# alexklibisz/deep-calcium

Hardware: NVIDIA B200
Metric: UNet2DS 512x512 images/sec (8x TTA) (higher is better)
Workload: dtype f16

## Files before the change

### deep-calcium_b200/csrc/core.cu

```cuda
#include "common.cuh"

namespace dcb {

unsigned long long g_launches = 0;

char* last_error_buf() {
  static thread_local char buf[512] = {0};
  return buf;
}

int fail(int code, const char* fmt, ...) {
  va_list ap;
  va_start(ap, fmt);
  vsnprintf(last_error_buf(), 512, fmt, ap);
  va_end(ap);
  return code;
}

int sm_count() {
  static int cached = 0;
  if (cached == 0) {
    int dev = 0, n = 0;
    if (cudaGetDevice(&dev) == cudaSuccess &&
        cudaDeviceGetAttribute(&n, cudaDevAttrMultiProcessorCount, dev) == cudaSuccess && n > 0)
      cached = n;
    else
      cached = 148;
  }
  return cached;
}

static const int kPolicyDefaults[DCB_POLICY_COUNT] = {
     1,  1,  1,  1,  64,  1,
     4,  0,  1,  2,  1,  1,  0,  0};
static int g_policy[DCB_POLICY_COUNT] = {1, 1, 1, 1, 64, 1, 4, 0, 1, 2, 1, 1, 0, 0};

int policy(int key) { return (key >= 0 && key < DCB_POLICY_COUNT) ? g_policy[key] : 0; }

char* last_kernel_buf() {
  static thread_local char buf[96] = {0};
  return buf;
}
void note_kernel(const char* name) {
  char* b = last_kernel_buf();
  strncpy(b, name, 95);
  b[95] = 0;
}

}

// ... 20 lines not shown
```

### deep-calcium_b200/csrc/tapgemm_tc.cu

```cuda
#include <cstdlib>
#include <mutex>
#include <map>
#include <vector>
#include <tuple>

#include "tc_common.cuh"
#include "stats_epilogue.cuh"
#include "tapgeom.h"

namespace dcb {
extern unsigned long long g_launches;
using namespace tc;

constexpr int TC_BM = 128;
constexpr int TC_MAX_STAGES = 8;
constexpr int TC_THREADS = 64 + 8 * 32;
constexpr int ST_QUARTETS = 2;
constexpr int ST_THREADS = 64 + ST_QUARTETS * 4 * 32;
constexpr int WG_THREADS = 192;

struct TcFusion {
  const float* head_kernel; const float* head_bias; float* logit; float* prob; int need_y; void* pool_out;
};

// ... 119 lines not shown
#pragma unroll
    for (int k = 0; k < 16; ++k) st[k * 32 + lane] = pooled[k];
    __syncwarp();
#pragma unroll
    for (int q = 0; q < 2; ++q) {
      const int idx = lane + 32 * q, pp = idx >> 2, chunk = idx & 3;
      const long long o = pool_index(m0 + 2 * pp);
      if (o >= 0)
        *reinterpret_cast<uint4*>(reinterpret_cast<uint16_t*>(pool_base) + o + chunk * 8) =
            *reinterpret_cast<const uint4*>(st + pp * 32 + chunk * 8);
    }
    __syncwarp();
  }
}

template <bool POOL, bool STATS>
__global__ void __launch_bounds__(TC_THREADS, 1)
tapgemm_tc_fwd_kernel(const __grid_constant__ CUtensorMap mapA0, const __grid_constant__ CUtensorMap mapA1,
                      const __grid_constant__ CUtensorMap mapB, const __grid_constant__ CUtensorMap mapO, const TcFwdParams p) {
  extern __shared__ __align__(1024) uint8_t smem_raw[];
  __shared__ uint64_t bar_full[TC_MAX_STAGES], bar_empty[TC_MAX_STAGES], bar_tfull[2], bar_tempty[2];
  __shared__ uint32_t tmem_base_smem;
  __shared__ __align__(16) float s_scale[512], s_shift[512];

  const int warp = threadIdx.x >> 5, lane = threadIdx.x & 31;
  if (threadIdx.x == 0) pdl_trigger();
  uint8_t* smem = smem_raw + ((1024u - (smem_u32(smem_raw) & 1023u)) & 1023u);
  const int PX = p.swap ? 256 : TC_BM;
  const uint32_t a_bytes = PX * p.BK * 2, b_bytes = (p.swap ? 128 : p.BN) * p.BK * 2;
  const uint32_t stage_bytes = a_bytes + b_bytes;
  const int kb0 = p.C0 / p.BK, kb1 = p.C1 / p.BK;
  const int kb_per_tap = kb0 + kb1;
  const int num_kb = p.ntaps * kb_per_tap;
  const int Ktap = p.C0 + p.C1;
  const int num_ntiles = p.swap ? (p.Ntot + 127) / 128 : p.Ntot / p.BN;
  const int num_mtiles = p.tiles_w * p.tiles_h * p.tiles_n;
  const int num_tiles = num_mtiles * num_ntiles;
  const int acc_cols = p.swap ? 256 : p.BN;
  uint32_t tmem_cols = 32;
  while (tmem_cols < 2u * acc_cols) tmem_cols <<= 1;
  __shared__ __align__(16) uint8_t s_stage[4][4096];
  float2 st_s[STATS ? 8 : 1], st_q[STATS ? 8 : 1];
#pragma unroll
  for (int i = 0; i < (STATS ? 8 : 1); ++i) { st_s[i] = make_float2(0.f, 0.f); st_q[i] = make_float2(0.f, 0.f); }

  for (int i = threadIdx.x; i < p.Cz; i += blockDim.x) {
    s_scale[i] = p.scale ? p.scale[i] : 1.f;
    s_shift[i] = p.shift ? p.shift[i] : 0.f;
  }
  if (warp == 0 && lane == 0) {
    tma_prefetch_desc(&mapA0);
    if (p.C1 > 0) tma_prefetch_desc(&mapA1);
    tma_prefetch_desc(&mapB);
    for (int s = 0; s < p.stages; ++s) { mbar_init(&bar_full[s], 1); mbar_init(&bar_empty[s], 1); }
    for (int s = 0; s < 2; ++s) { mbar_init(&bar_tfull[s], 1); mbar_init(&bar_tempty[s], 4); }
    mbar_fence_init();
  }
  if (warp == 1) {
    tmem_alloc(&tmem_base_smem, tmem_cols);
    tmem_relinquish();
  }
  tc_fence_before();
  __syncthreads();
  tc_fence_after();
  const uint32_t tmem_base = tmem_base_smem;

  if (warp == 0) {
    if (elect_one()) {
      int stage = 0; uint32_t phase = 0;
      pdl_wait();
      for (int tile = blockIdx.x; tile < num_tiles; tile += gridDim.x) {
        const int nt = tile % num_ntiles, mt = tile / num_ntiles;
        const int tw = mt % p.tiles_w, th = (mt / p.tiles_w) % p.tiles_h, tn = mt / (p.tiles_w * p.tiles_h);
        const int w0 = tw * p.bw, h0 = th * p.bh, n0 = tn * p.bn;
        for (int tap = 0; tap < p.ntaps; ++tap) {
          for (int kk = 0; kk < kb_per_tap; ++kk) {
            const bool second = kk >= kb0;
            const int c0 = (second ? kk - kb0 : kk) * p.BK;
            const CUtensorMap* mA = second ? &mapA1 : &mapA0;
            mbar_wait(&bar_empty[stage], phase ^ 1);
            uint8_t* sa = smem + (size_t)stage * stage_bytes;
            uint8_t* sb = sa + a_bytes;
            const int wrows = p.swap ? (p.Ntot - nt * 128 < 128 ? p.Ntot - nt * 128 : 128) : p.BN;
            mbar_arrive_expect_tx(&bar_full[stage], a_bytes + (uint32_t)wrows * p.BK * 2);
            if (p.mode == 0) tma_load_4d(mA, &bar_full[stage], sa, c0, w0 + p.dx[tap], h0 + p.dy[tap], n0);
            else if (p.mode == 1) tma_load_3d(mA, &bar_full[stage], sa, c0, w0, h0);
            else tma_load_5d(mA, &bar_full[stage], sa, c0, p.dx[tap], w0, p.dy[tap], h0);
            tma_load_2d(&mapB, &bar_full[stage], sb, tap * Ktap + (second ? p.C0 : 0) + c0, nt * (p.swap ? 128 : p.BN));
            if (++stage == p.stages) { stage = 0; phase ^= 1; }
          }
        }
      }
    }
  } else if (warp == 1) {
    if (elect_one()) {
      const uint32_t idesc = p.swap ? make_idesc_16(128, 256, 0, 0, p.f16) : make_idesc_16(TC_BM, p.BN, 0, 0, p.f16);
      const uint32_t swz = (p.BK == 64) ? SWZ_128B : SWZ_64B;
      const uint32_t sbo = 8u * p.BK * 2u;
      const int ksteps = p.BK / 16;
      const uint64_t dbase = make_smem_desc(0, 16, sbo, swz);
      const uint32_t smem16 = smem_u32(smem) >> 4, stage16 = stage_bytes >> 4, a16 = a_bytes >> 4;
      int stage = 0; uint32_t phase = 0;
      int acc = 0; uint32_t acc_phase = 0;
      const uint32_t a_full = smem_u32_pinned(bar_full), a_empty = smem_u32_pinned(bar_empty);
      asm volatile(".reg .pred p_full;");
      bool pre = false;
      for (int tile = blockIdx.x; tile < num_tiles; tile += gridDim.x) {
        mbar_wait(&bar_tempty[acc], acc_phase ^ 1);
        tc_fence_after();
        const uint32_t d_tmem = tmem_base + (uint32_t)(acc * acc_cols);
        for (int kb = 0; kb < num_kb; ++kb) {
          {
            uint32_t ok = 0;
            if (pre) asm volatile("selp.u32 %0, 1, 0, p_full;" : "=r"(ok));
            if (!ok) mbar_wait_a(a_full + 8u * stage, phase);
            int ns = stage + 1; uint32_t np = phase;
            if (ns == p.stages) { ns = 0; np ^= 1u; }
            asm volatile("mbarrier.test_wait.parity.shared::cta.b64 p_full, [%0], %1;" ::"r"(a_full + 8u * ns), "r"(np) : "memory");
            pre = true;
          }
          tc_fence_after();
          const uint32_t sa16 = smem16 + (uint32_t)stage * stage16, sb16 = sa16 + a16;
          const uint64_t da = dbase + (p.swap ? sb16 : sa16);
          const uint64_t db = dbase + (p.swap ? sa16 : sb16);
#pragma unroll
          for (int k = 0; k < 4; ++k) {
            if (k < ksteps) umma_bf16(d_tmem, da + (uint64_t)(2 * k), db + (uint64_t)(2 * k), idesc, (kb | k) != 0 ? 1u : 0u);
          }
          umma_commit_a(a_empty + 8u * stage);
          if (++stage == p.stages) { stage = 0; phase ^= 1; }
        }
        umma_commit(&bar_tfull[acc]);
        if (++acc == 2) { acc = 0; acc_phase ^= 1; }
      }
    }
  } else {
    const int quarter = warp & 3;
    const int m = quarter * 32 + lane;
    const int eset = (warp - 2) >> 2, nsets = p.swap ? 1 : 2;
    uint32_t it = 0;
    for (int tile = blockIdx.x; tile < num_tiles && eset < nsets; tile += gridDim.x, ++it) {
      if (nsets == 2 && (int)(it & 1u) != eset) continue;
      const int acc = (int)(it & 1u);
      const uint32_t acc_phase = (it >> 1) & 1u;
      const int nt = tile % num_ntiles, mt = tile / num_ntiles;
      const int tw = mt % p.tiles_w, th = (mt / p.tiles_w) % p.tiles_h, tn = mt / (p.tiles_w * p.tiles_h);
      if (p.swap) {
        const int grow = nt * 128 + quarter * 32;
        const bool warp_valid = grow < p.Ntot;
        const int z = grow / p.Cz, cw = grow % p.Cz;
        const int ody = p.Cz < p.Ntot ? (z >> 1) : p.ody, odx = p.Cz < p.Ntot ? (z & 1) : p.odx;
        const float sc = warp_valid ? s_scale[cw + lane] : 0.f, sh = warp_valid ? s_shift[cw + lane] : 0.f;
        auto pix_index = [&](int mm) -> long long {
          int n2, gh2, gw2;
          if (p.mode == 0) {
            gw2 = tw * p.bw + mm % p.bw;
            gh2 = th * p.bh + (mm / p.bw) % p.bh;
            n2 = tn * p.bn + mm / (p.bw * p.bh);
            if (gw2 >= p.GW || gh2 >= p.GH || n2 >= p.N) return -1;
          } else {
// ... 8 lines not shown
        tc_fence_after();
        if constexpr (POOL) {
          auto pool_index = [&](int mm) -> long long {
            const int gw2 = tw * p.bw + mm % p.bw, gh2 = th * p.bh + (mm / p.bw) % p.bh, n2 = tn * p.bn + mm / (p.bw * p.bh);
            if (gw2 >= p.GW || gh2 >= p.GH || n2 >= p.N) return -1;
            return (long long)((((size_t)n2 * (p.GH >> 1) + (gh2 >> 1)) * (p.GW >> 1) + (gw2 >> 1)) * p.OC + cw);
          };
          epilogue_swapped_pool(tmem_base + ((uint32_t)(quarter * 32) << 16) + (uint32_t)(acc * acc_cols), 256, p.bw, warp_valid, sc,
                                sh, p.relu, p.out, p.pool_out, s_stage[quarter], lane, pix_index, pool_index, p.f16);
        } else {
          epilogue_swapped(tmem_base + ((uint32_t)(quarter * 32) << 16) + (uint32_t)(acc * acc_cols), 256, warp_valid, sc, sh,
                           p.relu, p.out_f32, p.out, s_stage[quarter], lane, pix_index, p.f16);
        }
        tc_fence_before();
        __syncwarp();
        if (lane == 0) mbar_arrive(&bar_tempty[acc]);
        continue;
      }
      int n, gh, gw;
      bool valid;
      if (p.mode == 0) {
        gw = tw * p.bw + m % p.bw;
        gh = th * p.bh + (m / p.bw) % p.bh;
        n = tn * p.bn + m / (p.bw * p.bh);
        valid = gw < p.GW && gh < p.GH && n < p.N;
      } else {
        gw = tw * p.bw + m % p.bw;
        const int r = th * p.bh + m / p.bw;
        n = r / p.GH; gh = r % p.GH;
        valid = gw < p.GW && r < p.N * p.GH;
      }
// ... 137 lines not shown
              for (int q = 0; q < 4; ++q) {
                const uint4 b4 = stg[(m + 1) * 4 + q], c4 = stg[(m + p.bw) * 4 + q], d4 = stg[(m + p.bw + 1) * 4 + q];
                mx[4 * q] = max16x2(max16x2(pk[4 * q], b4.x, p.f16), max16x2(c4.x, d4.x, p.f16), p.f16);
                mx[4 * q + 1] = max16x2(max16x2(pk[4 * q + 1], b4.y, p.f16), max16x2(c4.y, d4.y, p.f16), p.f16);
                mx[4 * q + 2] = max16x2(max16x2(pk[4 * q + 2], b4.z, p.f16), max16x2(c4.z, d4.z, p.f16), p.f16);
                mx[4 * q + 3] = max16x2(max16x2(pk[4 * q + 3], b4.w, p.f16), max16x2(c4.w, d4.w, p.f16), p.f16);
              }
              store_pk16(p.pool_out + (((size_t)n * (p.GH >> 1) + (gh >> 1)) * (p.GW >> 1) + (gw >> 1)) * p.OC + cbase + c, mx);
            }
            asm volatile("bar.sync %0, 128;" ::"r"(1 + eset) : "memory");
          }
        }
      }
      tc_fence_before();
      __syncwarp();
      if (lane == 0) mbar_arrive(&bar_tempty[acc]);
    }
    if (p.tma_store && quarter == 0 && lane == 0) bulk_wait0();
  }

  tc_fence_before();
  __syncthreads();
  if (warp == 1) {
    tc_fence_after();
    tmem_dealloc(tmem_base, tmem_cols);
  }
  if constexpr (STATS) {
    float* dump = reinterpret_cast<float*>(smem);
    const int nblk = p.BN / 32;
    if (warp >= 2 && lane < 16) {
#pragma unroll
      for (int bi = 0; bi < 8; ++bi)
        if (bi < nblk)
          *reinterpret_cast<float4*>(dump + ((size_t)((warp - 2) * nblk + bi) * 16 + lane) * 4) =
              make_float4(st_s[bi].x, st_s[bi].y, st_q[bi].x, st_q[bi].y);
    }
    __syncthreads();
    const int nt = blockIdx.x % num_ntiles;
    stats_cta_finish(dump, 8, nblk, [&](int bi) { return (nt * p.BN + bi * 32) % p.Cz; }, p.Cz, p.stat_sums);
  }
// ... 46 lines not shown
  umma_bf16(d2, dA, dW + 2u * wblk16, id1, 0u);
  for (int kc = 0; kc < nkc; ++kc) {
#pragma unroll
    for (int dx = 0; dx < 3; ++dx) {
#pragma unroll
      for (int k = 0; k < KSTEPS; ++k) {
        if (kc == 0 && dx == 0 && k == 0) continue;
        umma_bf16(d0, dA + (kc * slot16 + dx * pitch16 + 2 * k), dW + ((uint32_t)(kc * 3 + dx) * 3u * wblk16 + 2 * k), id3, 1u);
      }
    }
  }
}

constexpr int ST_MAX_RING = 12;

__device__ __forceinline__ uint32_t cluster_ctarank() {
  uint32_t r;
  asm volatile("mov.u32 %0, %%cluster_ctarank;" : "=r"(r));
  return r;
}
__device__ __forceinline__ void cluster_sync_all() {
  asm volatile("barrier.cluster.arrive.release.aligned;" ::: "memory");
  asm volatile("barrier.cluster.wait.acquire.aligned;" ::: "memory");
}
__device__ __forceinline__ void tma_load_4d_mc(const CUtensorMap* m, uint64_t* bar, void* dst, int c0, int c1, int c2, int c3,
                                               uint16_t cta_mask) {
  asm volatile(
      "cp.async.bulk.tensor.4d.shared::cluster.global.mbarrier::complete_tx::bytes.multicast::cluster [%0], [%1, {%3, %4, %5, %6}], [%2], %7;"
      ::"r"(smem_u32(dst)), "l"(reinterpret_cast<uint64_t>(m)), "r"(smem_u32(bar)), "r"(c0), "r"(c1), "r"(c2), "r"(c3), "h"(cta_mask)
      : "memory");
}
__device__ __forceinline__ void umma_commit_mc2(uint32_t bar_addr) {
  asm volatile("tcgen05.commit.cta_group::1.mbarrier::arrive::one.shared::cluster.multicast::cluster.b64 [%0], %1;"
               ::"r"(bar_addr), "h"((uint16_t)3) : "memory");
}

#ifdef DCB_STRIP_TIMING
__device__ unsigned long long g_strip_dbg[148 * 8];
__device__ unsigned long long g_strip_dbg2[148 * 16];
// ... 641 lines not shown
    if (warp >= 2 && lane < 16) {
#pragma unroll
      for (int bi = 0; bi < 2; ++bi)
        if (bi < nblk)
          *reinterpret_cast<float4*>(dump + ((size_t)((warp - 2) * nblk + bi) * 16 + lane) * 4) =
              make_float4(sst.s[bi].x, sst.s[bi].y, sst.q[bi].x, sst.q[bi].y);
    }
    __syncthreads();
    stats_cta_finish(dump, 8, nblk, [](int bi) { return bi * 32; }, p.Cout, p.stat_sums);
  }
}

__device__ __forceinline__ uint32_t st2_region(int t0, int run) {
  return run == 3 ? 7u : (run == 2 ? (t0 == 0 ? 3u : 5u) : (uint32_t)t0);
}
__device__ __forceinline__ uint32_t mapa_u32(uint32_t addr, uint32_t rank) {
  uint32_t r;
  asm volatile("mapa.shared::cluster.u32 %0, %1, %2;" : "=r"(r) : "r"(addr), "r"(rank));
  return r;
}
__device__ __forceinline__ void mbar_arrive_cluster(uint32_t bar_addr) {
  asm volatile("mbarrier.arrive.relaxed.cluster.shared::cluster.b64 _, [%0];" ::"r"(bar_addr) : "memory");
}
__device__ __forceinline__ void mbar_arrive_expect_tx_cluster(uint32_t bar_addr, uint32_t bytes) {
  asm volatile("mbarrier.arrive.expect_tx.relaxed.cluster.shared::cluster.b64 _, [%0], %1;" ::"r"(bar_addr), "r"(bytes) : "memory");
}
__device__ __forceinline__ void tma_load_2d_pair(const CUtensorMap* m, uint32_t bar_addr, void* dst, int c0, int c1) {
  asm volatile(
      "cp.async.bulk.tensor.2d.shared::cluster.global.mbarrier::complete_tx::bytes.cta_group::2 [%0], [%1, {%3, %4}], [%2];"
      ::"r"(smem_u32(dst)), "l"(reinterpret_cast<uint64_t>(m)), "r"(bar_addr), "r"(c0), "r"(c1) : "memory");
}
__device__ __forceinline__ void tma_load_4d_pair(const CUtensorMap* m, uint32_t bar_addr, void* dst, int c0, int c1, int c2, int c3) {
  asm volatile(
      "cp.async.bulk.tensor.4d.shared::cluster.global.mbarrier::complete_tx::bytes.cta_group::2 [%0], [%1, {%3, %4, %5, %6}], [%2];"
      ::"r"(smem_u32(dst)), "l"(reinterpret_cast<uint64_t>(m)), "r"(bar_addr), "r"(c0), "r"(c1), "r"(c2), "r"(c3) : "memory");
}
__device__ __forceinline__ void umma2_bf16(uint32_t tmem_d, uint64_t desc_a, uint64_t desc_b, uint32_t idesc, uint32_t accumulate) {
  asm volatile(
      "{\n\t.reg .pred p;\n\t"
      "setp.ne.b32 p, %4, 0;\n\t"
      "tcgen05.mma.cta_group::2.kind::f16 [%0], %1, %2, %3, p;\n\t}"
      ::"r"(tmem_d), "l"(desc_a), "l"(desc_b), "r"(idesc), "r"(accumulate) : "memory");
}
__device__ __forceinline__ void umma2_commit_both(uint32_t bar_addr) {
  asm volatile("tcgen05.commit.cta_group::2.mbarrier::arrive::one.shared::cluster.multicast::cluster.b64 [%0], %1;"
               ::"r"(bar_addr), "h"((uint16_t)3) : "memory");
}

template <int KSTEPS>
__device__ __forceinline__ void fold2_issue_fast(uint32_t d0, uint32_t d2, uint64_t dA, uint64_t dW, uint32_t id1, uint32_t id2,
                                                 uint32_t id3, int nkc, uint32_t slot16, uint32_t pitch16, uint32_t half16,
                                                 uint32_t group16) {
  umma2_bf16(d0, dA, dW + 3u * half16, id2, 1u);
  umma2_bf16(d2, dA, dW + 2u * half16, id1, 0u);
  const uint64_t dW3 = dW + 7u * half16;
  for (int kc = 0; kc < nkc; ++kc) {
#pragma unroll
    for (int dx = 0; dx < 3; ++dx) {
#pragma unroll
      for (int k = 0; k < KSTEPS; ++k) {
        if (kc == 0 && dx == 0 && k == 0) continue;
        umma2_bf16(d0, dA + (kc * slot16 + dx * pitch16 + 2 * k), dW3 + ((uint32_t)(kc * 3 + dx) * group16 + 2 * k), id3, 1u);
// ... 28 lines not shown

  for (int i = threadIdx.x; i < p.Cout; i += blockDim.x) {
    s_scale[i] = p.scale ? p.scale[p.n0 + i] : 1.f;
    s_shift[i] = p.shift ? p.shift[p.n0 + i] : 0.f;
    s_wd[i] = p.head_kernel ? p.head_kernel[2 * i + 1] - p.head_kernel[2 * i] : 0.f;
  }
  if (warp == 0 && lane == 0) {
    tma_prefetch_desc(&mapA0);
    if (p.C1 > 0) tma_prefetch_desc(&mapA1);
    tma_prefetch_desc(&mapBh);
    mbar_init(&bar_w, 2);
    for (int s = 0; s < ring_pairs; ++s) { mbar_init(&row_full[s], 2); mbar_init(&row_empty[s], 1); }
    for (int s = 0; s < (nacc >> 1); ++s) { mbar_init(&bar_tfull[s], 1); mbar_init(&bar_tempty[s], 8); }
    mbar_fence_init();
  }
  if (warp == 1) {
    asm volatile("tcgen05.alloc.cta_group::2.sync.aligned.shared::cta.b32 [%0], %1;" ::"r"(smem_u32(&tmem_base_smem)), "r"(512u) : "memory");
    asm volatile("tcgen05.relinquish_alloc_permit.cta_group::2.sync.aligned;" ::: "memory");
  }
  tc_fence_before();
  cluster_sync_all();
  tc_fence_after();
  const uint32_t tmem_base = tmem_base_smem;

  const int units_per_col = p.H >> 1;
  const int npairs = gridDim.x >> 1, pair = blockIdx.x >> 1;
  const long long units = (long long)(p.N * p.wsegs / 2) * units_per_col;
  const long long u_begin = units * pair / npairs, u_end = units * (pair + 1) / npairs;
  auto next_strip = [&](long long& u, int& n, int& h0, int& rows, int& w0) -> bool {
    if (u >= u_end) return false;
    const int pcol = (int)(u / units_per_col), hu = (int)(u - (long long)pcol * units_per_col);
    long long take = units_per_col - hu;
    if (take > u_end - u) take = u_end - u;
    const int col = 2 * pcol + (int)rank;
// ... 173 lines not shown
        const uint32_t ta = t_lane + (j & (uint32_t)(nacc - 1)) * (uint32_t)p.Cout, tb = ta + (uint32_t)p.Cout;
        const int bar_i = (int)(jp & pmask);
        mbar_wait(&bar_tfull[bar_i], (j >> nacc_sh) & 1u);
        tc_fence_after();
        strip_drain_pair<FUSED>(p, ta, tb, n, h0 + t, w0 + m, s_scale, s_shift, s_wd, head_b, lane, p.n0);
        tc_fence_before();
        __syncwarp();
        if (lane == 0) mbar_arrive_cluster(l_tempty + 8u * bar_i);
      }
    }
  }
  tc_fence_before();
  cluster_sync_all();
  if (warp == 1) {
    tc_fence_after();
    asm volatile("tcgen05.dealloc.cta_group::2.sync.aligned.b32 %0, %1;" ::"r"(tmem_base), "r"(512u) : "memory");
  }
}

struct TcFlatParams {
  int N, H, W, Wp;
  int C0, C1, nkc;
  int Cout, mtiles;
  int NT, ptiles;
  int R;
  int wrows;
  uint32_t pbuf_bytes;
  int relu, out_f32;
  int f16;
  void* out;
  const float* scale;
// ... 517 lines not shown
                e[1], e[0] / e[1], e[3], e[2] / e[3], e[4] / e[3], e[5] / e[3], e[6] / e[3], e[8], e[7] / e[8], e[9] / e[8], e[10] / e[8], e[11] / e[8]);
        fprintf(stderr, "[strip timing] per CTA: fast rows %.0f | cycles/row: row_full wait %.0f, tempty wait %.0f, issue %.0f, commit %.0f, "
                "total %.0f | loop cycles %.0f\n", a[5], a[0] / a[5], a[1] / a[5], a[2] / a[5], a[3] / a[5], a[4] / a[5], a[6]);
      }
#endif
      return DCB_OK;
    }
  }
  if (!(stats && stats->sums && policy(DCB_POLICY_FUSED_BN) == 2)) {
    const int e = run_tc_flat(g, s0, C0, s1, C1, B, Nout, out, scale, shift, relu, out_f32, st, stats);
    if (e != DCB_ERR_UNSUPPORTED) return e;
  }
  return run_tc_generic(g, s0, C0, s1, C1, B, Nout, out, Nout, scale, shift, relu, out_f32, st, nullptr, stats);
}

static int run_tc_generic(const TapGeom& g, const void* s0, int C0, const void* s1, int C1, const void* B, int Nout, void* out,
                          int out_pitch, const float* scale, const float* shift, int relu, int out_f32, cudaStream_t st,
                          void* pool_out, TcStats* stats) {
  TcFwdParams p;
  memset(&p, 0, sizeof(p));
  const int ntaps = g.ntaps;
  const bool convT_fwd = g.zsub > 1;
  const bool convT_dgrad = (g.sy == 2);
  p.mode = convT_fwd ? 1 : (convT_dgrad ? 2 : 0);
  p.N = g.N; p.GH = g.GH; p.GW = g.GW;
  p.ntaps = ntaps;
  for (int t = 0; t < ntaps; ++t) { p.dy[t] = g.dy[t]; p.dx[t] = g.dx[t]; }
  p.C0 = C0; p.C1 = C1;
  p.BK = (C0 % 64 == 0 && C1 % 64 == 0) ? 64 : 32;
  const int swz = p.BK * 2;
  p.Cz = Nout;
  p.Ntot = convT_fwd ? 4 * Nout : Nout;
  p.OH = g.OH; p.OW = g.OW; p.OC = out_pitch;
  p.osy = g.osy; p.osx = g.osx; p.ody = g.ody; p.odx = g.odx;
  p.relu = relu; p.out_f32 = out_f32; p.out = reinterpret_cast<__nv_bfloat16*>(out); p.scale = scale; p.shift = shift;
  p.f16 = g.f16;
  {
    const long long px = (long long)g.N * g.GH * g.GW;
    p.swap = (p.mode == 0 && !pool_out && !stats && swap_allowed(Nout) && px / 256 * cdiv(p.Ntot, 128) >= sm_count() / 2) ? 1 : 0;
  }
  const int TM = p.swap ? 256 : TC_BM;
  if (p.mode == 0) {
    p.bw = pick_pow2_box(g.GW, TM);
    if (pool_out && p.bw == TM && TM >= 4) p.bw = TM / 2;
    p.bh = pick_pow2_box(g.GH, TM / p.bw);
    p.bn = TM / (p.bw * p.bh);
    p.tiles_w = cdiv(g.GW, p.bw); p.tiles_h = cdiv(g.GH, p.bh); p.tiles_n = cdiv(g.N, p.bn);
  } else {
    p.bw = pick_pow2_box(g.GW, TM);
    p.bh = TM / p.bw; p.bn = 1;
    p.tiles_w = cdiv(g.GW, p.bw); p.tiles_h = cdiv((long long)g.N * g.GH, p.bh); p.tiles_n = 1;
  }
  const int num_mtiles = p.tiles_w * p.tiles_h * p.tiles_n;
  if (pool_out) {
    if (p.mode != 0 || out_f32 || (g.GH & 1) || (g.GW & 1) || (p.bw & 1) || (p.bh & 1) || (p.swap && p.bw % 32 != 0) || out_pitch != Nout)
      return fail(DCB_ERR_UNSUPPORTED, "fused max-pool not available for this layer shape");
    p.pool_out = reinterpret_cast<__nv_bfloat16*>(pool_out);
  }
  int BN = 32;
  {
    double best = 1e30;
    for (int cand : {256, 192, 128, 96, 64, 32}) {
      if (cand > p.Ntot || p.Ntot % cand != 0) continue;
      const long long tiles = (long long)num_mtiles * (p.Ntot / cand);
      const long long waves = (tiles + sm_count() - 1) / sm_count();
      const double cost = (double)waves * (cand <= 128 ? 89.0 : 89.0 + (cand - 128) * (39.0 / 128.0));
      if (cost < best - 1e-9) { best = cost; BN = cand; }
    }
  }
  if (p.swap) BN = p.Ntot < 128 ? p.Ntot : 128;
  p.BN = BN;
  const size_t stage_bytes = (size_t)TM * p.BK * 2 + (size_t)(p.swap ? 128 : BN) * p.BK * 2;
  const bool with_stats = stats && !pool_out && !out_f32 && p.mode != 2 && out_pitch == Nout && stats->sums;
  p.tma_store = (!p.swap && !out_f32 && !pool_out && !with_stats && p.mode != 2 &&
                 (policy(DCB_POLICY_TMA_STORE) >= 2 || (policy(DCB_POLICY_TMA_STORE) == 1 && p.mode == 1))) ? 1 : 0;
  const size_t staging = p.tma_store ? 2 * 16384 : 0;
  int stages = (int)((200 * 1024 - staging) / stage_bytes);
  if (stages > TC_MAX_STAGES) stages = TC_MAX_STAGES;
  if (stages < 2) return fail(DCB_ERR_UNSUPPORTED, "tile does not fit shared memory");
  p.stages = stages;
  const size_t dyn_smem = stages * stage_bytes + staging + 1024;

  CUtensorMap mA0, mA1, mB;
  auto make_src_map = [&](CUtensorMap* m, const void* ptr, int C) -> int {
    if (p.mode == 0) {
      uint64_t dims[4] = {(uint64_t)C, (uint64_t)g.IW, (uint64_t)g.IH, (uint64_t)g.N};
      uint64_t str[3] = {(uint64_t)C * 2, (uint64_t)g.IW * C * 2, (uint64_t)g.IH * g.IW * C * 2};
      uint32_t box[4] = {(uint32_t)p.BK, (uint32_t)p.bw, (uint32_t)p.bh, (uint32_t)p.bn};
      return make_map(m, ptr, 4, dims, str, box, swz);
// ... 4 lines not shown
      return make_map(m, ptr, 3, dims, str, box, swz);
    } else {
      uint64_t dims[5] = {(uint64_t)C, 2, (uint64_t)g.GW, 2, (uint64_t)g.N * g.GH};
      uint64_t str[4] = {(uint64_t)C * 2, (uint64_t)2 * C * 2, (uint64_t)g.IW * C * 2, (uint64_t)2 * g.IW * C * 2};
      uint32_t box[5] = {(uint32_t)p.BK, 1, (uint32_t)p.bw, 1, (uint32_t)p.bh};
      return make_map(m, ptr, 5, dims, str, box, swz);
    }
  };
  if (int e = make_src_map(&mA0, s0, C0)) return e;
  if (C1 > 0) { if (int e = make_src_map(&mA1, s1, C1)) return e; }
  else mA1 = mA0;
  {
    const int Ktot = ntaps * (C0 + C1);
    uint64_t dims[2] = {(uint64_t)Ktot, (uint64_t)p.Ntot};
    uint64_t str[1] = {(uint64_t)Ktot * 2};
    uint32_t box[2] = {(uint32_t)p.BK, (uint32_t)BN};
    if (int e = make_map(&mB, B, 2, dims, str, box, swz)) return e;
  }

  CUtensorMap mO = mB;
  if (p.tma_store) {
    if (p.mode == 0) {
      uint64_t dims[4] = {(uint64_t)Nout, (uint64_t)g.OW, (uint64_t)g.OH, (uint64_t)g.N};
      uint64_t str[3] = {(uint64_t)out_pitch * 2, (uint64_t)g.OW * out_pitch * 2, (uint64_t)g.OH * g.OW * out_pitch * 2};
      uint32_t box[4] = {32u, (uint32_t)p.bw, (uint32_t)p.bh, (uint32_t)p.bn};
      if (int e = make_map(&mO, out, 4, dims, str, box, 64)) return e;
    } else {
      uint64_t dims[5] = {(uint64_t)Nout, 2, (uint64_t)g.GW, 2, (uint64_t)g.N * g.GH};
      uint64_t str[4] = {(uint64_t)out_pitch * 2, (uint64_t)2 * out_pitch * 2, (uint64_t)g.OW * out_pitch * 2,
                         (uint64_t)2 * g.OW * out_pitch * 2};
      uint32_t box[5] = {32u, 1, (uint32_t)p.bw, 1, (uint32_t)p.bh};
      if (int e = make_map(&mO, out, 5, dims, str, box, 64)) return e;
    }
  }
  static bool attr_set = false;
  if (!attr_set) {
    cudaError_t e = cudaFuncSetAttribute(tapgemm_tc_fwd_kernel<false, false>, cudaFuncAttributeMaxDynamicSharedMemorySize, 206 * 1024);
    if (e == cudaSuccess) e = cudaFuncSetAttribute(tapgemm_tc_fwd_kernel<true, false>, cudaFuncAttributeMaxDynamicSharedMemorySize, 206 * 1024);
    if (e == cudaSuccess) e = cudaFuncSetAttribute(tapgemm_tc_fwd_kernel<false, true>, cudaFuncAttributeMaxDynamicSharedMemorySize, 206 * 1024);
    if (e != cudaSuccess) return fail(DCB_ERR_CUDA, "cudaFuncSetAttribute(max dynamic smem) failed: %s", cudaGetErrorString(e));
    attr_set = true;
  }
  const int num_ntiles = p.swap ? cdiv(p.Ntot, 128) : p.Ntot / BN;
  const int num_tiles = num_mtiles * num_ntiles;
  int grid = num_tiles < sm_count() ? num_tiles : sm_count();
  const bool pdl = policy(DCB_POLICY_PDL) != 0;
  if (with_stats) {
    grid -= grid % num_ntiles;
    if (grid >= num_ntiles) {
      p.stat_sums = stats->sums;
      const cudaError_t le = launch_k(tapgemm_tc_fwd_kernel<false, true>, grid, TC_THREADS, dyn_smem, st, pdl, mA0, mA1, mB, mO, p);
      if (le != cudaSuccess) return fail(DCB_ERR_CUDA, "launch of tapgemm_tc_fwd_kernel (stats) failed: %s", cudaGetErrorString(le));
      g_launches += 1;
      stats->done = 1;
      note_kernel("generic_stats");
      return DCB_OK;
    }
    grid = num_tiles < sm_count() ? num_tiles : sm_count();
  }
  {
    const cudaError_t le = p.pool_out ? launch_k(tapgemm_tc_fwd_kernel<true, false>, grid, TC_THREADS, dyn_smem, st, pdl, mA0, mA1, mB, mO, p)
// ... 509 lines not shown
```

### deep-calcium_b200/deepcalcium/_native.py

```python
import ctypes
import os

_HERE = os.path.dirname(os.path.abspath(__file__))
LIB_PATH = os.path.join(_HERE, '_lib', 'libdcb200.so')

_lib = None

c_int = ctypes.c_int
c_ll = ctypes.c_longlong
c_f = ctypes.c_float
c_d = ctypes.c_double
c_p = ctypes.c_void_p
c_sz = ctypes.c_size_t

DCB_F32, DCB_BF16, DCB_F16 = 0, 1, 2
POLICY_KEYS = {'flat': 0, 'strip': 1, 'fold': 2, 'nsplit': 3, 'swap_min_cout': 4, 'wgrad_strip': 5, 'bn_ctas_per_sm': 6,
               'proj_i16_splits': 7, 'splitk': 8, 'fused_bn': 9, 'tma_store': 10, 'bn_slab': 11, 'pdl': 12, 'pair': 13}
LOSS_IDS = {'binary_crossentropy': 0, 'weighted_binary_crossentropy': 1, 'dice_loss': 2, 'dicesq_loss': 3}


class DcbError(RuntimeError):
    pass


def lib():
    global _lib
    if _lib is None:
        if not os.path.exists(LIB_PATH):
            raise DcbError('libdcb200.so not built (%s); run `python deep-calcium_b200/build.py` or '
                           '__graft_entry__.build() - there is no CPU fallback' % LIB_PATH)
        _lib = ctypes.CDLL(LIB_PATH)
        _lib.dcb_last_error.restype = ctypes.c_char_p
# ... 73 lines not shown
```

### include/dcb200.h

```cpp
#ifndef DCB200_H_
#define DCB200_H_

#include <stddef.h>
#include <stdint.h>

#ifdef __cplusplus
extern "C" {
#endif

typedef void* dcb_stream_t;

enum dcb_status {
  DCB_OK = 0,
  DCB_ERR_INVALID_ARGUMENT = -1,
  DCB_ERR_CUDA = -2,
  DCB_ERR_WORKSPACE = -3,
  DCB_ERR_UNSUPPORTED = -4
};

enum dcb_dtype { DCB_F32 = 0, DCB_BF16 = 1, DCB_F16 = 2 };

enum dcb_loss { DCB_LOSS_BCE = 0, DCB_LOSS_WBCE = 1, DCB_LOSS_DICE = 2, DCB_LOSS_DICESQ = 3 };

int dcb_version(void);
// ... 3 lines not shown
enum dcb_policy_key {
  DCB_POLICY_FLAT = 0,
  DCB_POLICY_STRIP = 1,
  DCB_POLICY_FOLD = 2,
  DCB_POLICY_NSPLIT = 3,
  DCB_POLICY_SWAP_MIN_COUT = 4,
  DCB_POLICY_WGRAD_STRIP = 5,
  DCB_POLICY_BN_CTAS_PER_SM = 6,
  DCB_POLICY_PROJ_I16_SPLITS = 7,
  DCB_POLICY_SPLITK = 8,
  DCB_POLICY_FUSED_BN = 9,
  DCB_POLICY_TMA_STORE = 10,
  DCB_POLICY_BN_SLAB = 11,
  DCB_POLICY_PDL = 12,
  DCB_POLICY_PAIR = 13,
  DCB_POLICY_COUNT = 14
};
int dcb_set_policy(int key, int value);
int dcb_get_policy(int key, int* value);
int dcb_reset_policy(void);
const char* dcb_last_kernel(void);

int dcb_proj_workspace_bytes(int T, int H, int W, size_t* bytes);
int dcb_proj_mean_max_f32(const float* movie, int T, int H, int W, float* mean, float* max,
                          int floor_max_at_zero, void* workspace, size_t workspace_bytes,
                          dcb_stream_t stream);
int dcb_proj_mean_max_f32_variant(const float* movie, int T, int H, int W, float* mean, float* max,
                                  int floor_max_at_zero, void* workspace, size_t workspace_bytes,
                                  int variant, int t_splits, dcb_stream_t stream);

int dcb_proj_mean_max_i16(const short* movie, int T, int H, int W, float* mean, float* mx, int floor_max_at_zero, void* workspace,
// ... 165 lines not shown
```

Before: 1097.

## Add CTA-pair (cta_group::2) path to generic tap-GEMM forward kernel

Result: faster. 1114 (median of 6 runs) (+1.5%).

```diff
diff --git a/deep-calcium_b200/csrc/core.cu b/deep-calcium_b200/csrc/core.cu
--- a/deep-calcium_b200/csrc/core.cu
+++ b/deep-calcium_b200/csrc/core.cu
@@ -32,8 +32,9 @@
 
 static const int kPolicyDefaults[DCB_POLICY_COUNT] = {
      1,  1,  1,  1,  64,  1,
-     4,  0,  1,  2,  1,  1,  0,  0};
-static int g_policy[DCB_POLICY_COUNT] = {1, 1, 1, 1, 64, 1, 4, 0, 1, 2, 1, 1, 0, 0};
+     4,  0,  1,  2,  1,  1,  0,  0,
+     1};
+static int g_policy[DCB_POLICY_COUNT] = {1, 1, 1, 1, 64, 1, 4, 0, 1, 2, 1, 1, 0, 0, 1};
 
 int policy(int key) { return (key >= 0 && key < DCB_POLICY_COUNT) ? g_policy[key] : 0; }
 
diff --git a/deep-calcium_b200/csrc/tapgemm_tc.cu b/deep-calcium_b200/csrc/tapgemm_tc.cu
--- a/deep-calcium_b200/csrc/tapgemm_tc.cu
+++ b/deep-calcium_b200/csrc/tapgemm_tc.cu
@@ -157,7 +157,56 @@
   }
 }
 
-template <bool POOL, bool STATS>
+__device__ __forceinline__ uint32_t cluster_ctarank() {
+  uint32_t r;
+  asm volatile("mov.u32 %0, %%cluster_ctarank;" : "=r"(r));
+  return r;
+}
+__device__ __forceinline__ void cluster_sync_all() {
+  asm volatile("barrier.cluster.arrive.release.aligned;" ::: "memory");
+  asm volatile("barrier.cluster.wait.acquire.aligned;" ::: "memory");
+}
+__device__ __forceinline__ uint32_t mapa_u32(uint32_t addr, uint32_t rank) {
+  uint32_t r;
+  asm volatile("mapa.shared::cluster.u32 %0, %1, %2;" : "=r"(r) : "r"(addr), "r"(rank));
+  return r;
+}
+__device__ __forceinline__ void mbar_arrive_cluster(uint32_t bar_addr) {
+  asm volatile("mbarrier.arrive.relaxed.cluster.shared::cluster.b64 _, [%0];" ::"r"(bar_addr) : "memory");
+}
+__device__ __forceinline__ void mbar_arrive_expect_tx_cluster(uint32_t bar_addr, uint32_t bytes) {
+  asm volatile("mbarrier.arrive.expect_tx.relaxed.cluster.shared::cluster.b64 _, [%0], %1;" ::"r"(bar_addr), "r"(bytes) : "memory");
+}
+__device__ __forceinline__ void tma_load_2d_pair(const CUtensorMap* m, uint32_t bar_addr, void* dst, int c0, int c1) {
+  asm volatile(
+      "cp.async.bulk.tensor.2d.shared::cluster.global.mbarrier::complete_tx::bytes.cta_group::2 [%0], [%1, {%3, %4}], [%2];"
+      ::"r"(smem_u32(dst)), "l"(reinterpret_cast<uint64_t>(m)), "r"(bar_addr), "r"(c0), "r"(c1) : "memory");
+}
+__device__ __forceinline__ void tma_load_4d_pair(const CUtensorMap* m, uint32_t bar_addr, void* dst, int c0, int c1, int c2, int c3) {
+  asm volatile(
+      "cp.async.bulk.tensor.4d.shared::cluster.global.mbarrier::complete_tx::bytes.cta_group::2 [%0], [%1, {%3, %4, %5, %6}], [%2];"
+      ::"r"(smem_u32(dst)), "l"(reinterpret_cast<uint64_t>(m)), "r"(bar_addr), "r"(c0), "r"(c1), "r"(c2), "r"(c3) : "memory");
+}
+__device__ __forceinline__ void umma2_bf16(uint32_t tmem_d, uint64_t desc_a, uint64_t desc_b, uint32_t idesc, uint32_t accumulate) {
+  asm volatile(
+      "{\n\t.reg .pred p;\n\t"
+      "setp.ne.b32 p, %4, 0;\n\t"
+      "tcgen05.mma.cta_group::2.kind::f16 [%0], %1, %2, %3, p;\n\t}"
+      ::"r"(tmem_d), "l"(desc_a), "l"(desc_b), "r"(idesc), "r"(accumulate) : "memory");
+}
+__device__ __forceinline__ void umma2_commit_both(uint32_t bar_addr) {
+  asm volatile("tcgen05.commit.cta_group::2.mbarrier::arrive::one.shared::cluster.multicast::cluster.b64 [%0], %1;"
+               ::"r"(bar_addr), "h"((uint16_t)3) : "memory");
+}
+__device__ __forceinline__ void tmem_alloc_pair(uint32_t* dst, uint32_t ncols) {
+  asm volatile("tcgen05.alloc.cta_group::2.sync.aligned.shared::cta.b32 [%0], %1;" ::"r"(smem_u32(dst)), "r"(ncols) : "memory");
+  asm volatile("tcgen05.relinquish_alloc_permit.cta_group::2.sync.aligned;" ::: "memory");
+}
+__device__ __forceinline__ void tmem_dealloc_pair(uint32_t base, uint32_t ncols) {
+  asm volatile("tcgen05.dealloc.cta_group::2.sync.aligned.b32 %0, %1;" ::"r"(base), "r"(ncols) : "memory");
+}
+
+template <bool POOL, bool STATS, bool PAIR = false>
 __global__ void __launch_bounds__(TC_THREADS, 1)
 tapgemm_tc_fwd_kernel(const __grid_constant__ CUtensorMap mapA0, const __grid_constant__ CUtensorMap mapA1,
                       const __grid_constant__ CUtensorMap mapB, const __grid_constant__ CUtensorMap mapO, const TcFwdParams p) {
@@ -166,11 +215,13 @@
   __shared__ uint32_t tmem_base_smem;
   __shared__ __align__(16) float s_scale[512], s_shift[512];
 
+  static_assert(!(PAIR && STATS), "the statistics epilogue keeps the single-CTA kernel");
   const int warp = threadIdx.x >> 5, lane = threadIdx.x & 31;
   if (threadIdx.x == 0) pdl_trigger();
+  const uint32_t rank = PAIR ? cluster_ctarank() : 0u;
   uint8_t* smem = smem_raw + ((1024u - (smem_u32(smem_raw) & 1023u)) & 1023u);
   const int PX = p.swap ? 256 : TC_BM;
-  const uint32_t a_bytes = PX * p.BK * 2, b_bytes = (p.swap ? 128 : p.BN) * p.BK * 2;
+  const uint32_t a_bytes = PX * p.BK * 2, b_bytes = (p.swap ? 128 : (PAIR ? p.BN / 2 : p.BN)) * p.BK * 2;
   const uint32_t stage_bytes = a_bytes + b_bytes;
   const int kb0 = p.C0 / p.BK, kb1 = p.C1 / p.BK;
   const int kb_per_tap = kb0 + kb1;
@@ -178,7 +229,9 @@
   const int Ktap = p.C0 + p.C1;
   const int num_ntiles = p.swap ? (p.Ntot + 127) / 128 : p.Ntot / p.BN;
   const int num_mtiles = p.tiles_w * p.tiles_h * p.tiles_n;
-  const int num_tiles = num_mtiles * num_ntiles;
+  const int num_units = PAIR ? ((num_mtiles + 1) >> 1) * num_ntiles : num_mtiles * num_ntiles;
+  const int u_first = PAIR ? (int)(blockIdx.x >> 1) : (int)blockIdx.x, u_step = PAIR ? (int)(gridDim.x >> 1) : (int)gridDim.x;
+  auto unit_mtile = [&](int u) { return PAIR ? 2 * (u / num_ntiles) + (int)rank : u / num_ntiles; };
   const int acc_cols = p.swap ? 256 : p.BN;
   uint32_t tmem_cols = 32;
   while (tmem_cols < 2u * acc_cols) tmem_cols <<= 1;
@@ -195,25 +248,31 @@
     tma_prefetch_desc(&mapA0);
     if (p.C1 > 0) tma_prefetch_desc(&mapA1);
     tma_prefetch_desc(&mapB);
-    for (int s = 0; s < p.stages; ++s) { mbar_init(&bar_full[s], 1); mbar_init(&bar_empty[s], 1); }
-    for (int s = 0; s < 2; ++s) { mbar_init(&bar_tfull[s], 1); mbar_init(&bar_tempty[s], 4); }
+    for (int s = 0; s < p.stages; ++s) { mbar_init(&bar_full[s], PAIR ? 2 : 1); mbar_init(&bar_empty[s], 1); }
+    for (int s = 0; s < 2; ++s) { mbar_init(&bar_tfull[s], 1); mbar_init(&bar_tempty[s], PAIR ? 8 : 4); }
     mbar_fence_init();
   }
   if (warp == 1) {
-    tmem_alloc(&tmem_base_smem, tmem_cols);
-    tmem_relinquish();
+    if constexpr (PAIR) {
+      tmem_alloc_pair(&tmem_base_smem, tmem_cols);
+    } else {
+      tmem_alloc(&tmem_base_smem, tmem_cols);
+      tmem_relinquish();
+    }
   }
   tc_fence_before();
-  __syncthreads();
+  if constexpr (PAIR) cluster_sync_all();
+  else __syncthreads();
   tc_fence_after();
   const uint32_t tmem_base = tmem_base_smem;
 
   if (warp == 0) {
     if (elect_one()) {
       int stage = 0; uint32_t phase = 0;
+      const uint32_t l_full = PAIR ? mapa_u32(smem_u32(bar_full), 0) : 0u;
       pdl_wait();
-      for (int tile = blockIdx.x; tile < num_tiles; tile += gridDim.x) {
-        const int nt = tile % num_ntiles, mt = tile / num_ntiles;
+      for (int tile = u_first; tile < num_units; tile += u_step) {
+        const int nt = tile % num_ntiles, mt = unit_mtile(tile);
         const int tw = mt % p.tiles_w, th = (mt / p.tiles_w) % p.tiles_h, tn = mt / (p.tiles_w * p.tiles_h);
         const int w0 = tw * p.bw, h0 = th * p.bh, n0 = tn * p.bn;
         for (int tap = 0; tap < p.ntaps; ++tap) {
@@ -224,6 +283,15 @@
             mbar_wait(&bar_empty[stage], phase ^ 1);
             uint8_t* sa = smem + (size_t)stage * stage_bytes;
             uint8_t* sb = sa + a_bytes;
+            if constexpr (PAIR) {
+              const uint32_t lf = l_full + 8u * stage;
+              const bool has_a = mt < num_mtiles;
+              mbar_arrive_expect_tx_cluster(lf, (has_a ? a_bytes : 0u) + b_bytes);
+              if (has_a) tma_load_4d_pair(mA, lf, sa, c0, w0 + p.dx[tap], h0 + p.dy[tap], n0);
+              tma_load_2d_pair(&mapB, lf, sb, tap * Ktap + (second ? p.C0 : 0) + c0, nt * p.BN + (int)rank * (p.BN >> 1));
+              if (++stage == p.stages) { stage = 0; phase ^= 1; }
+              continue;
+            }
             const int wrows = p.swap ? (p.Ntot - nt * 128 < 128 ? p.Ntot - nt * 128 : 128) : p.BN;
             mbar_arrive_expect_tx(&bar_full[stage], a_bytes + (uint32_t)wrows * p.BK * 2);
             if (p.mode == 0) tma_load_4d(mA, &bar_full[stage], sa, c0, w0 + p.dx[tap], h0 + p.dy[tap], n0);
@@ -236,8 +304,8 @@
       }
     }
   } else if (warp == 1) {
-    if (elect_one()) {
-      const uint32_t idesc = p.swap ? make_idesc_16(128, 256, 0, 0, p.f16) : make_idesc_16(TC_BM, p.BN, 0, 0, p.f16);
+    if ((!PAIR || rank == 0) && elect_one()) {
+      const uint32_t idesc = p.swap ? make_idesc_16(128, 256, 0, 0, p.f16) : make_idesc_16(PAIR ? 2 * TC_BM : TC_BM, p.BN, 0, 0, p.f16);
       const uint32_t swz = (p.BK == 64) ? SWZ_128B : SWZ_64B;
       const uint32_t sbo = 8u * p.BK * 2u;
       const int ksteps = p.BK / 16;
@@ -248,7 +316,7 @@
       const uint32_t a_full = smem_u32_pinned(bar_full), a_empty = smem_u32_pinned(bar_empty);
       asm volatile(".reg .pred p_full;");
       bool pre = false;
-      for (int tile = blockIdx.x; tile < num_tiles; tile += gridDim.x) {
+      for (int tile = u_first; tile < num_units; tile += u_step) {
         mbar_wait(&bar_tempty[acc], acc_phase ^ 1);
         tc_fence_after();
         const uint32_t d_tmem = tmem_base + (uint32_t)(acc * acc_cols);
@@ -268,12 +336,17 @@
           const uint64_t db = dbase + (p.swap ? sa16 : sb16);
 #pragma unroll
           for (int k = 0; k < 4; ++k) {
-            if (k < ksteps) umma_bf16(d_tmem, da + (uint64_t)(2 * k), db + (uint64_t)(2 * k), idesc, (kb | k) != 0 ? 1u : 0u);
-          }
-          umma_commit_a(a_empty + 8u * stage);
+            if (k < ksteps) {
+              if constexpr (PAIR) umma2_bf16(d_tmem, da + (uint64_t)(2 * k), db + (uint64_t)(2 * k), idesc, (kb | k) != 0 ? 1u : 0u);
+              else umma_bf16(d_tmem, da + (uint64_t)(2 * k), db + (uint64_t)(2 * k), idesc, (kb | k) != 0 ? 1u : 0u);
+            }
+          }
+          if constexpr (PAIR) umma2_commit_both(a_empty + 8u * stage);
+          else umma_commit_a(a_empty + 8u * stage);
           if (++stage == p.stages) { stage = 0; phase ^= 1; }
         }
-        umma_commit(&bar_tfull[acc]);
+        if constexpr (PAIR) umma2_commit_both(smem_u32(&bar_tfull[acc]));
+        else umma_commit(&bar_tfull[acc]);
         if (++acc == 2) { acc = 0; acc_phase ^= 1; }
       }
     }
@@ -281,12 +354,17 @@
     const int quarter = warp & 3;
     const int m = quarter * 32 + lane;
     const int eset = (warp - 2) >> 2, nsets = p.swap ? 1 : 2;
+    const uint32_t l_tempty = PAIR ? mapa_u32(smem_u32(bar_tempty), 0) : 0u;
+    auto release_acc = [&](int acc) {
+      if constexpr (PAIR) mbar_arrive_cluster(l_tempty + 8u * acc);
+      else mbar_arrive(&bar_tempty[acc]);
+    };
     uint32_t it = 0;
-    for (int tile = blockIdx.x; tile < num_tiles && eset < nsets; tile += gridDim.x, ++it) {
+    for (int tile = u_first; tile < num_units && eset < nsets; tile += u_step, ++it) {
       if (nsets == 2 && (int)(it & 1u) != eset) continue;
       const int acc = (int)(it & 1u);
       const uint32_t acc_phase = (it >> 1) & 1u;
-      const int nt = tile % num_ntiles, mt = tile / num_ntiles;
+      const int nt = tile % num_ntiles, mt = unit_mtile(tile);
       const int tw = mt % p.tiles_w, th = (mt / p.tiles_w) % p.tiles_h, tn = mt / (p.tiles_w * p.tiles_h);
       if (p.swap) {
         const int grow = nt * 128 + quarter * 32;
@@ -325,7 +403,7 @@
         }
         tc_fence_before();
         __syncwarp();
-        if (lane == 0) mbar_arrive(&bar_tempty[acc]);
+        if (lane == 0) release_acc(acc);
         continue;
       }
       int n, gh, gw;
@@ -493,16 +571,18 @@
       }
       tc_fence_before();
       __syncwarp();
-      if (lane == 0) mbar_arrive(&bar_tempty[acc]);
+      if (lane == 0) release_acc(acc);
     }
     if (p.tma_store && quarter == 0 && lane == 0) bulk_wait0();
   }
 
   tc_fence_before();
-  __syncthreads();
+  if constexpr (PAIR) cluster_sync_all();
+  else __syncthreads();
   if (warp == 1) {
     tc_fence_after();
-    tmem_dealloc(tmem_base, tmem_cols);
+    if constexpr (PAIR) tmem_dealloc_pair(tmem_base, tmem_cols);
+    else tmem_dealloc(tmem_base, tmem_cols);
   }
   if constexpr (STATS) {
     float* dump = reinterpret_cast<float*>(smem);
@@ -579,15 +659,6 @@
 
 constexpr int ST_MAX_RING = 12;
 
-__device__ __forceinline__ uint32_t cluster_ctarank() {
-  uint32_t r;
-  asm volatile("mov.u32 %0, %%cluster_ctarank;" : "=r"(r));
-  return r;
-}
-__device__ __forceinline__ void cluster_sync_all() {
-  asm volatile("barrier.cluster.arrive.release.aligned;" ::: "memory");
-  asm volatile("barrier.cluster.wait.acquire.aligned;" ::: "memory");
-}
 __device__ __forceinline__ void tma_load_4d_mc(const CUtensorMap* m, uint64_t* bar, void* dst, int c0, int c1, int c2, int c3,
                                                uint16_t cta_mask) {
   asm volatile(
@@ -1259,38 +1330,6 @@
 __device__ __forceinline__ uint32_t st2_region(int t0, int run) {
   return run == 3 ? 7u : (run == 2 ? (t0 == 0 ? 3u : 5u) : (uint32_t)t0);
 }
-__device__ __forceinline__ uint32_t mapa_u32(uint32_t addr, uint32_t rank) {
-  uint32_t r;
-  asm volatile("mapa.shared::cluster.u32 %0, %1, %2;" : "=r"(r) : "r"(addr), "r"(rank));
-  return r;
-}
-__device__ __forceinline__ void mbar_arrive_cluster(uint32_t bar_addr) {
-  asm volatile("mbarrier.arrive.relaxed.cluster.shared::cluster.b64 _, [%0];" ::"r"(bar_addr) : "memory");
-}
-__device__ __forceinline__ void mbar_arrive_expect_tx_cluster(uint32_t bar_addr, uint32_t bytes) {
-  asm volatile("mbarrier.arrive.expect_tx.relaxed.cluster.shared::cluster.b64 _, [%0], %1;" ::"r"(bar_addr), "r"(bytes) : "memory");
-}
-__device__ __forceinline__ void tma_load_2d_pair(const CUtensorMap* m, uint32_t bar_addr, void* dst, int c0, int c1) {
-  asm volatile(
-      "cp.async.bulk.tensor.2d.shared::cluster.global.mbarrier::complete_tx::bytes.cta_group::2 [%0], [%1, {%3, %4}], [%2];"
-      ::"r"(smem_u32(dst)), "l"(reinterpret_cast<uint64_t>(m)), "r"(bar_addr), "r"(c0), "r"(c1) : "memory");
-}
-__device__ __forceinline__ void tma_load_4d_pair(const CUtensorMap* m, uint32_t bar_addr, void* dst, int c0, int c1, int c2, int c3) {
-  asm volatile(
-      "cp.async.bulk.tensor.4d.shared::cluster.global.mbarrier::complete_tx::bytes.cta_group::2 [%0], [%1, {%3, %4, %5, %6}], [%2];"
-      ::"r"(smem_u32(dst)), "l"(reinterpret_cast<uint64_t>(m)), "r"(bar_addr), "r"(c0), "r"(c1), "r"(c2), "r"(c3) : "memory");
-}
-__device__ __forceinline__ void umma2_bf16(uint32_t tmem_d, uint64_t desc_a, uint64_t desc_b, uint32_t idesc, uint32_t accumulate) {
-  asm volatile(
-      "{\n\t.reg .pred p;\n\t"
-      "setp.ne.b32 p, %4, 0;\n\t"
-      "tcgen05.mma.cta_group::2.kind::f16 [%0], %1, %2, %3, p;\n\t}"
-      ::"r"(tmem_d), "l"(desc_a), "l"(desc_b), "r"(idesc), "r"(accumulate) : "memory");
-}
-__device__ __forceinline__ void umma2_commit_both(uint32_t bar_addr) {
-  asm volatile("tcgen05.commit.cta_group::2.mbarrier::arrive::one.shared::cluster.multicast::cluster.b64 [%0], %1;"
-               ::"r"(bar_addr), "h"((uint16_t)3) : "memory");
-}
 
 template <int KSTEPS>
 __device__ __forceinline__ void fold2_issue_fast(uint32_t d0, uint32_t d2, uint64_t dA, uint64_t dW, uint32_t id1, uint32_t id2,
@@ -1349,10 +1388,7 @@
     for (int s = 0; s < (nacc >> 1); ++s) { mbar_init(&bar_tfull[s], 1); mbar_init(&bar_tempty[s], 8); }
     mbar_fence_init();
   }
-  if (warp == 1) {
-    asm volatile("tcgen05.alloc.cta_group::2.sync.aligned.shared::cta.b32 [%0], %1;" ::"r"(smem_u32(&tmem_base_smem)), "r"(512u) : "memory");
-    asm volatile("tcgen05.relinquish_alloc_permit.cta_group::2.sync.aligned;" ::: "memory");
-  }
+  if (warp == 1) tmem_alloc_pair(&tmem_base_smem, 512u);
   tc_fence_before();
   cluster_sync_all();
   tc_fence_after();
@@ -1556,7 +1592,7 @@
   cluster_sync_all();
   if (warp == 1) {
     tc_fence_after();
-    asm volatile("tcgen05.dealloc.cta_group::2.sync.aligned.b32 %0, %1;" ::"r"(tmem_base), "r"(512u) : "memory");
+    tmem_dealloc_pair(tmem_base, 512u);
   }
 }
 
@@ -2104,6 +2140,10 @@
   return run_tc_generic(g, s0, C0, s1, C1, B, Nout, out, Nout, scale, shift, relu, out_f32, st, nullptr, stats);
 }
 
+static bool pair_generic_pays(long long px, int K, int Nout) {
+  return px >= 2 * TC_BM && ((Nout == 256 && K >= 256) || (Nout == 128 && K == 128));
+}
+
 static int run_tc_generic(const TapGeom& g, const void* s0, int C0, const void* s1, int C1, const void* B, int Nout, void* out,
                           int out_pitch, const float* scale, const float* shift, int relu, int out_f32, cudaStream_t st,
                           void* pool_out, TcStats* stats) {
@@ -2125,10 +2165,14 @@
   p.osy = g.osy; p.osx = g.osx; p.ody = g.ody; p.odx = g.odx;
   p.relu = relu; p.out_f32 = out_f32; p.out = reinterpret_cast<__nv_bfloat16*>(out); p.scale = scale; p.shift = shift;
   p.f16 = g.f16;
-  {
-    const long long px = (long long)g.N * g.GH * g.GW;
-    p.swap = (p.mode == 0 && !pool_out && !stats && swap_allowed(Nout) && px / 256 * cdiv(p.Ntot, 128) >= sm_count() / 2) ? 1 : 0;
-  }
+  const bool with_stats = stats && !pool_out && !out_f32 && p.mode != 2 && out_pitch == Nout && stats->sums;
+  const long long px = (long long)g.N * g.GH * g.GW;
+  bool pair = false;
+  if (p.mode == 0 && !out_f32 && !with_stats && policy(DCB_POLICY_TMA_STORE) < 2 && sm_count() >= 2) {
+    const int pp = policy(DCB_POLICY_PAIR_GENERIC);
+    pair = pp >= 2 || (pp == 1 && pair_generic_pays(px, C0 + C1, Nout));
+  }
+  p.swap = (!pair && p.mode == 0 && !pool_out && !stats && swap_allowed(Nout) && px / 256 * cdiv(p.Ntot, 128) >= sm_count() / 2) ? 1 : 0;
   const int TM = p.swap ? 256 : TC_BM;
   if (p.mode == 0) {
     p.bw = pick_pow2_box(g.GW, TM);
@@ -2149,20 +2193,24 @@
   }
   int BN = 32;
   {
+    const long long units_m = pair ? (num_mtiles + 1) / 2 : num_mtiles;
+    const int slots = pair ? sm_count() / 2 : sm_count();
     double best = 1e30;
     for (int cand : {256, 192, 128, 96, 64, 32}) {
       if (cand > p.Ntot || p.Ntot % cand != 0) continue;
-      const long long tiles = (long long)num_mtiles * (p.Ntot / cand);
-      const long long waves = (tiles + sm_count() - 1) / sm_count();
-      const double cost = (double)waves * (cand <= 128 ? 89.0 : 89.0 + (cand - 128) * (39.0 / 128.0));
+      const long long tiles = units_m * (p.Ntot / cand);
+      const long long waves = (tiles + slots - 1) / slots;
+      const double c = pair ? (cand <= 64 ? 48.0 : (cand <= 128 ? 48.0 + (cand - 64) * 0.25 : 64.0 + (cand - 128) * 0.5))
+                            : (cand <= 128 ? 89.0 : 89.0 + (cand - 128) * (39.0 / 128.0));
+      const double cost = (double)waves * c;
       if (cost < best - 1e-9) { best = cost; BN = cand; }
     }
   }
   if (p.swap) BN = p.Ntot < 128 ? p.Ntot : 128;
   p.BN = BN;
-  const size_t stage_bytes = (size_t)TM * p.BK * 2 + (size_t)(p.swap ? 128 : BN) * p.BK * 2;
-  const bool with_stats = stats && !pool_out && !out_f32 && p.mode != 2 && out_pitch == Nout && stats->sums;
-  p.tma_store = (!p.swap && !out_f32 && !pool_out && !with_stats && p.mode != 2 &&
+  const int brows = p.swap ? 128 : (pair ? BN / 2 : BN);
+  const size_t stage_bytes = (size_t)TM * p.BK * 2 + (size_t)brows * p.BK * 2;
+  p.tma_store = (!pair && !p.swap && !out_f32 && !pool_out && !with_stats && p.mode != 2 &&
                  (policy(DCB_POLICY_TMA_STORE) >= 2 || (policy(DCB_POLICY_TMA_STORE) == 1 && p.mode == 1))) ? 1 : 0;
   const size_t staging = p.tma_store ? 2 * 16384 : 0;
   int stages = (int)((200 * 1024 - staging) / stage_bytes);
@@ -2197,7 +2245,7 @@
     const int Ktot = ntaps * (C0 + C1);
     uint64_t dims[2] = {(uint64_t)Ktot, (uint64_t)p.Ntot};
     uint64_t str[1] = {(uint64_t)Ktot * 2};
-    uint32_t box[2] = {(uint32_t)p.BK, (uint32_t)BN};
+    uint32_t box[2] = {(uint32_t)p.BK, (uint32_t)(pair ? BN / 2 : BN)};
     if (int e = make_map(&mB, B, 2, dims, str, box, swz)) return e;
   }
 
@@ -2221,6 +2269,8 @@
     cudaError_t e = cudaFuncSetAttribute(tapgemm_tc_fwd_kernel<false, false>, cudaFuncAttributeMaxDynamicSharedMemorySize, 206 * 1024);
     if (e == cudaSuccess) e = cudaFuncSetAttribute(tapgemm_tc_fwd_kernel<true, false>, cudaFuncAttributeMaxDynamicSharedMemorySize, 206 * 1024);
     if (e == cudaSuccess) e = cudaFuncSetAttribute(tapgemm_tc_fwd_kernel<false, true>, cudaFuncAttributeMaxDynamicSharedMemorySize, 206 * 1024);
+    if (e == cudaSuccess) e = cudaFuncSetAttribute(tapgemm_tc_fwd_kernel<false, false, true>, cudaFuncAttributeMaxDynamicSharedMemorySize, 206 * 1024);
+    if (e == cudaSuccess) e = cudaFuncSetAttribute(tapgemm_tc_fwd_kernel<true, false, true>, cudaFuncAttributeMaxDynamicSharedMemorySize, 206 * 1024);
     if (e != cudaSuccess) return fail(DCB_ERR_CUDA, "cudaFuncSetAttribute(max dynamic smem) failed: %s", cudaGetErrorString(e));
     attr_set = true;
   }
@@ -2228,6 +2278,15 @@
   const int num_tiles = num_mtiles * num_ntiles;
   int grid = num_tiles < sm_count() ? num_tiles : sm_count();
   const bool pdl = policy(DCB_POLICY_PDL) != 0;
+  if (pair) {
+    const int units = (num_mtiles + 1) / 2 * num_ntiles, pairs = units < sm_count() / 2 ? units : sm_count() / 2;
+    const cudaError_t le = p.pool_out ? launch_kc(tapgemm_tc_fwd_kernel<true, false, true>, 2 * pairs, TC_THREADS, dyn_smem, st, pdl, 2, mA0, mA1, mB, mO, p)
+                                      : launch_kc(tapgemm_tc_fwd_kernel<false, false, true>, 2 * pairs, TC_THREADS, dyn_smem, st, pdl, 2, mA0, mA1, mB, mO, p);
+    if (le != cudaSuccess) return fail(DCB_ERR_CUDA, "launch of tapgemm_tc_fwd_kernel (pair) failed: %s", cudaGetErrorString(le));
+    g_launches += 1;
+    note_kernel(p.pool_out ? "generic_pair_pool" : "generic_pair");
+    return DCB_OK;
+  }
   if (with_stats) {
     grid -= grid % num_ntiles;
     if (grid >= num_ntiles) {
diff --git a/deep-calcium_b200/deepcalcium/_native.py b/deep-calcium_b200/deepcalcium/_native.py
--- a/deep-calcium_b200/deepcalcium/_native.py
+++ b/deep-calcium_b200/deepcalcium/_native.py
@@ -15,7 +15,8 @@
 
 DCB_F32, DCB_BF16, DCB_F16 = 0, 1, 2
 POLICY_KEYS = {'flat': 0, 'strip': 1, 'fold': 2, 'nsplit': 3, 'swap_min_cout': 4, 'wgrad_strip': 5, 'bn_ctas_per_sm': 6,
-               'proj_i16_splits': 7, 'splitk': 8, 'fused_bn': 9, 'tma_store': 10, 'bn_slab': 11, 'pdl': 12, 'pair': 13}
+               'proj_i16_splits': 7, 'splitk': 8, 'fused_bn': 9, 'tma_store': 10, 'bn_slab': 11, 'pdl': 12, 'pair': 13,
+               'pair_generic': 14}
 LOSS_IDS = {'binary_crossentropy': 0, 'weighted_binary_crossentropy': 1, 'dice_loss': 2, 'dicesq_loss': 3}
 
 
diff --git a/include/dcb200.h b/include/dcb200.h
--- a/include/dcb200.h
+++ b/include/dcb200.h
@@ -41,7 +41,8 @@
   DCB_POLICY_BN_SLAB = 11,
   DCB_POLICY_PDL = 12,
   DCB_POLICY_PAIR = 13,
-  DCB_POLICY_COUNT = 14
+  DCB_POLICY_PAIR_GENERIC = 14,
+  DCB_POLICY_COUNT = 15
 };
 int dcb_set_policy(int key, int value);
 int dcb_get_policy(int key, int* value);
```
